# simonamtoft/downsampled-diffusion

Measured on AMD Instinct MI355X. Metric: images/sec (T=1000 sampling), 256x256 dDDPM-x3, higher is better.
Workload: dtype f32

## Files before the change

downsampled-diffusion_amd/csrc/attention.hip:

```cpp
#include <cstdlib>

#include "cluster_sync.h"
#include "conv_common.h"

namespace ddk {

constexpr int DH = 32;

constexpr int PART = DH + DH + DH * DH;

__global__ __launch_bounds__(256) void linattn_context_kernel(const float* __restrict__ qkv, float* __restrict__ ctx,
                                                              float* __restrict__ part, int HW, int heads, int splits, int rows_per_split,
                                                              int kv_only) {
    __shared__ __attribute__((aligned(16))) float stage[4 * 32 * 33];
    float* kexp = stage;
    float* vs = stage + 64 * DH;
    __shared__ float smax[8 * DH];
    const int bh = blockIdx.x / splits, sp = blockIdx.x % splits;
    const int b = bh / heads, h = bh % heads;
    const int HC = heads * DH, RS = (kv_only ? 2 : 3) * HC;
    const float* base = qkv + (long long)b * HW * RS;
    const float* kp = base + (kv_only ? 0 : HC) + h * DH;
    const float* vp = kp + HC;
    const int tid = threadIdx.x;
// ... 1138 lines not shown
        for (int r = 0; r < 16; ++r) Ab[((r & 3) + 8 * (r >> 2) + 4 * kh) * FOLD_C] = acc[r];
        if (tid < 32) {
            float u1 = 0.f, u2 = 0.f;
#pragma unroll 16
            for (int he = 0; he < FOLD_C; ++he) {
                u1 += Wq[tid * (FOLD_C + 1) + he] * t1[he];
                u2 += Wq[tid * (FOLD_C + 1) + he] * t2[he];
            }
            const int n = nq * 32 + tid;
            a1[(long long)b * FOLD_C + n] = u1;
            a2[(long long)b * FOLD_C + n] = u2 + (bout ? bout[n] : 0.f);
        }
    }
}

int linattn_small_qkv_init_device() {
    DDK_HIP(hipFuncSetAttribute(reinterpret_cast<const void*>(attn_kvctx_kernel), hipFuncAttributeMaxDynamicSharedMemorySize,
                                (int)(KC_LDS_FLOATS * sizeof(float))));
    DDK_HIP(hipFuncSetAttribute(reinterpret_cast<const void*>(attn_fold_kernel), hipFuncAttributeMaxDynamicSharedMemorySize,
                                (int)(FOLD_LDS_FLOATS * sizeof(float))));
    DDK_HIP(hipFuncSetAttribute(reinterpret_cast<const void*>(linattn_small_kernel<256>), hipFuncAttributeMaxDynamicSharedMemorySize, 160 * 1024));
    DDK_HIP(hipFuncSetAttribute(reinterpret_cast<const void*>(linattn_small_qkv_kernel<1>), hipFuncAttributeMaxDynamicSharedMemorySize, 160 * 1024));
    DDK_HIP(hipFuncSetAttribute(reinterpret_cast<const void*>(linattn_small_qkv_kernel<4>), hipFuncAttributeMaxDynamicSharedMemorySize, 160 * 1024));
    DDK_HIP(hipFuncSetAttribute(reinterpret_cast<const void*>(attn_split_kernel<128>), hipFuncAttributeMaxDynamicSharedMemorySize,
                                (int)(AttnSplitGeom<128>::LDS_FL * sizeof(float))));
    DDK_HIP(hipFuncSetAttribute(reinterpret_cast<const void*>(attn_split_kernel<32>), hipFuncAttributeMaxDynamicSharedMemorySize,
                                (int)(AttnSplitGeom<32>::LDS_FL * sizeof(float))));
    return DDK_OK;
}

// ... 17 lines not shown
    else
        hipLaunchKernelGGL(linattn_small_qkv_kernel<4>, dim3(B * heads), dim3(256), small_qkv_lds_bytes(4, C), st, x, wop, c1, c2, ln_eps, ctx, out,
                           HW, C, heads);
    return check_launch("linattn_small_qkv_kernel");
}

bool attn_kvctx_ok(int B, int HW, int C, int heads) { return B > 0 && C == KC_K && heads == 4 && HW >= 4 * KC_BM && HW % KC_BM == 0; }
int attn_kvctx_splits(int B, int HW) {
    const int tiles = HW / KC_BM;
    int s = 1;
    while (s * 2 <= tiles && tiles % (s * 2) == 0 && (long long)B * 2 * (s * 2) <= 256) s *= 2;
    return s;
}
size_t attn_kvctx_workspace_bytes(int B, int HW) { return (size_t)B * 4 * attn_kvctx_splits(B, HW) * PART * sizeof(float); }

int attn_kvctx(const float* x, const float* w_kv, const float* c1, const float* c2, float ln_eps, float* ctx, int B, int HW, void* workspace,
               size_t workspace_bytes, hipStream_t st) {
    DDK_REQUIRE(x && w_kv && c1 && c2 && ctx && workspace, "attn_kvctx: null pointer");
    DDK_REQUIRE(attn_kvctx_ok(B, HW, KC_K, 4), "attn_kvctx: needs 128 channels, 4 heads, H*W a multiple of 64 and >= 256");
    DDK_REQUIRE(aligned16(x) && aligned16(w_kv) && aligned16(c1) && aligned16(c2) && aligned16(ctx) && aligned16(workspace), "attn_kvctx: alignment");
    DDK_REQUIRE((long long)B * HW * KC_K * 4 < (1LL << 32) && B <= 65535, "attn_kvctx: input of 4 GiB or more, or more than 65535 images");
    const int s = attn_kvctx_splits(B, HW);
    if (workspace_bytes < attn_kvctx_workspace_bytes(B, HW)) {
        set_error("attn_kvctx: workspace too small (%zu < %zu)", workspace_bytes, attn_kvctx_workspace_bytes(B, HW));
        return DDK_ERR_WORKSPACE;
    }
    DDK_TRY(ensure_device_init());
    KvCtxParams p{x, w_kv, c1, c2, ln_eps, static_cast<float*>(workspace), HW / KC_BM, HW / KC_BM / s, s};
    hipLaunchKernelGGL(attn_kvctx_kernel, dim3((unsigned)s, 2, (unsigned)B), dim3(512), KC_LDS_FLOATS * sizeof(float), st, p);
    DDK_TRY(check_launch("attn_kvctx_kernel"));
    hipLaunchKernelGGL(linattn_merge_kernel, dim3(B * 4), dim3(256), 0, st, static_cast<const float*>(workspace), ctx, s);
    return check_launch("linattn_merge_kernel");
}

constexpr int AS_CUS = 256;
bool attn_split_ok(int B, int HW, int C, int heads) {
    return B > 0 && (HW == 64 || HW == 256) && C >= 32 && C <= 256 && C % 32 == 0 && heads == 4 && 8 * (long long)B <= AS_CUS &&
           conv_wino_cluster_device_ok();
}
size_t attn_split_counter_words(int B) { return (size_t)B * 4 * AS_CNT; }
size_t attn_split_record_floats(int B) { return (size_t)B * 4 * 2 * AS_REC; }
size_t attn_split_workspace_bytes(int B) { return B > 0 ? (32 + attn_split_counter_words(B) + attn_split_record_floats(B)) * sizeof(float) : 0; }
unsigned attention_cluster_timeouts() { return cl_timeouts_read(); }

int attn_split(const float* x, const float* w, const float* c1, const float* c2, float ln_eps, float* ctx, float* out, int B, int HW, int C,
               unsigned* counters, float* records, unsigned* fail, hipStream_t st) {
// ... 10 lines not shown
}

bool attn_fold_ok(int C, int heads) { return C == FOLD_C && heads * DH == FOLD_C; }
size_t attn_fold_out_floats(int B) { return (size_t)B * (FOLD_C * FOLD_C + 2 * FOLD_C); }

int attn_fold(const float* ctx, const float* wqg, const float* c1q, const float* c2q, const float* wout, const float* bout, float* A,
              float* a1, float* a2, int B, int C, int heads, hipStream_t st) {
    DDK_REQUIRE(ctx && wqg && c1q && c2q && wout && A && a1 && a2 && B > 0, "attn_fold: arguments");
    DDK_REQUIRE(attn_fold_ok(C, heads), "attn_fold: C == 128 and heads * 32 == 128 only");
    DDK_REQUIRE(aligned16(ctx) && aligned16(wout) && aligned16(A), "attn_fold: alignment");
    DDK_TRY(ensure_device_init());
    hipLaunchKernelGGL(attn_fold_kernel, dim3(B, 4), dim3(256), FOLD_LDS_FLOATS * sizeof(float), st, ctx, wqg, c1q, c2q, wout, bout, A, a1, a2);
    return check_launch("attn_fold_kernel");
}

int linattn_apply(const float* qkv, const float* ctx, float* out, int B, int HW, int heads, hipStream_t st) {
    DDK_REQUIRE(qkv && ctx && out && B > 0 && HW > 0, "linattn_apply: arguments");
    DDK_REQUIRE(heads >= 1 && heads <= 8, "linattn_apply: heads must be in 1..8");
    DDK_REQUIRE(aligned16(qkv) && aligned16(ctx) && aligned16(out), "linattn_apply: alignment");
    const int tiles = (int)ceil_div(HW, 64);
    const size_t lds = (size_t)heads * 64 * 33 * sizeof(float);
    hipLaunchKernelGGL(linattn_apply_kernel, dim3(B * tiles), dim3(64 * heads), lds, st, qkv, ctx, out, HW, heads, tiles);
    return check_launch("linattn_apply_kernel");
}

}

extern "C" {
size_t ddk_linattn_context_workspace_bytes(int B, int HW, int heads) { return ddk::linattn_context_workspace_bytes(B, HW, heads); }
int ddk_linattn_context(const float* qkv, float* ctx, int B, int HW, int heads, void* workspace, size_t workspace_bytes, ddk_stream_t s) {
    return ddk::linattn_context(qkv, ctx, B, HW, heads, workspace, workspace_bytes, ddk::as_stream(s), false);
}
int ddk_linattn_context_kv(const float* kv, float* ctx, int B, int HW, int heads, void* workspace, size_t workspace_bytes, ddk_stream_t s) {
    return ddk::linattn_context(kv, ctx, B, HW, heads, workspace, workspace_bytes, ddk::as_stream(s), true);
}
size_t ddk_attention_kv_context_workspace_bytes(int B, int HW) { return ddk::attn_kvctx_workspace_bytes(B, HW); }
int ddk_attention_kv_context_ok(int B, int HW, int C, int heads) { return ddk::attn_kvctx_ok(B, HW, C, heads) ? 1 : 0; }
int ddk_attention_kv_context(const float* x, const float* w_kv, const float* c1, const float* c2, float ln_eps, float* ctx, int B, int HW,
                             void* workspace, size_t workspace_bytes, ddk_stream_t s) {
    return ddk::attn_kvctx(x, w_kv, c1, c2, ln_eps, ctx, B, HW, workspace, workspace_bytes, ddk::as_stream(s));
}
size_t ddk_attention_split_workspace_bytes(int B) { return ddk::attn_split_workspace_bytes(B); }
int ddk_attention_split_ok(int B, int HW, int C, int heads) { return ddk::attn_split_ok(B, HW, C, heads) ? 1 : 0; }
int ddk_attention_split_from_x(const float* x, const float* w_folded, const float* c1, const float* c2, float ln_eps, float* ctx, float* out,
                               int B, int HW, int C, int heads, void* workspace, size_t workspace_bytes, ddk_stream_t s) {
    using namespace ddk;
    DDK_REQUIRE(workspace && B > 0 && heads == 4, "attention_split_from_x: arguments (4 heads)");
    if (workspace_bytes < attn_split_workspace_bytes(B)) {
        set_error("attention_split_from_x: workspace too small (%zu < %zu)", workspace_bytes, attn_split_workspace_bytes(B));
        return DDK_ERR_WORKSPACE;
    }
    unsigned* words = static_cast<unsigned*>(workspace);
    return attn_split(x, w_folded, c1, c2, ln_eps, ctx, out, B, HW, C, words + 32, static_cast<float*>(workspace) + 32 + attn_split_counter_words(B),
                      words, as_stream(s));
}
// ... 19 lines not shown
```

downsampled-diffusion_amd/csrc/ddk_internal.h:

```cpp
#pragma once
#include <hip/hip_runtime.h>

#include <cstdarg>
#include <cstddef>
#include <cstdint>
#include <cstdio>

#include "ddk.h"

#ifdef DDK_HOST_SANITIZE
#include "host_sanitize.h"
#endif

namespace ddk {

void set_error(const char* fmt, ...);

inline int fail_arg(const char* what) {
    set_error("bad argument: %s", what);
    return DDK_ERR_ARG;
}

inline int check_launch(const char* what) {
    hipError_t e = hipGetLastError();
// ... 197 lines not shown
int groupnorm_mish_generic(const float* x, const float* gamma, const float* beta, const float* temb, int temb_stride, const float* addend,
                           float* out, int B, int HW, int CP, int C, int groups, float eps, hipStream_t st, const long long* temb_rows = nullptr);
int chan_layernorm_generic(const float* x, const float* g, const float* b, float* out, long long M, int CP, int C, float eps, hipStream_t st);
int unary(int op, const float* x, float* out, long long n, hipStream_t st);
int add(const float* a, const float* b, float* out, long long n, hipStream_t st);
int avgpool2(const float* x, float* out, int B, int H, int W, int C, hipStream_t st);
int upsample_nearest2(const float* x, float* out, int B, int H, int W, int C, hipStream_t st);
size_t linattn_context_workspace_bytes(int B, int HW, int heads);
int linattn_context(const float* qkv, float* ctx, int B, int HW, int heads, void* workspace, size_t workspace_bytes, hipStream_t st,
                    bool kv_only = false);
bool attn_fold_ok(int C, int heads);
bool attn_kvctx_ok(int B, int HW, int C, int heads);
size_t attn_kvctx_workspace_bytes(int B, int HW);
int attn_kvctx(const float* x, const float* w_kv, const float* c1, const float* c2, float ln_eps, float* ctx, int B, int HW, void* workspace,
               size_t workspace_bytes, hipStream_t st);
size_t attn_fold_out_floats(int B);
int attn_fold(const float* ctx, const float* wqg, const float* c1q, const float* c2q, const float* wout, const float* bout, float* A,
              float* a1, float* a2, int B, int C, int heads, hipStream_t st);
int linattn_apply(const float* qkv, const float* ctx, float* out, int B, int HW, int heads, hipStream_t st);
int linattn_fused_small(const float* qkv, float* ctx, float* out, int B, int HW, int heads, hipStream_t st);
bool attn_split_ok(int B, int HW, int C, int heads);
size_t attn_split_counter_words(int B);
size_t attn_split_record_floats(int B);
int attn_split(const float* x, const float* w, const float* c1, const float* c2, float ln_eps, float* ctx, float* out, int B, int HW, int C,
               unsigned* counters, float* records, unsigned* fail, hipStream_t st);
bool linattn_small_qkv_ok(int HW, int C);
int linattn_small_qkv_init_device();
int qkv_operand_pack(const float* lnw, float* wop, int heads, int cp, hipStream_t st);
int linattn_small_qkv(const float* x, const float* wop, const float* c1, const float* c2, float ln_eps, float* ctx, float* out, int B, int HW,
                      int C, int heads, hipStream_t st);
// ... 164 lines not shown
```

downsampled-diffusion_amd/csrc/unet_plan.hip:

```cpp
#include <algorithm>
#include <initializer_list>
#include <mutex>
#include <string>
#include <vector>

#include "ddk_internal.h"
#include "level_chain.h"

namespace ddk {

constexpr int HEADS = 4;
constexpr int HIDDEN = HEADS * 32;
constexpr int GROUPS = 8;
constexpr float GN_EPS = 1e-5f, LN_EPS = 1e-5f;

static inline int pad32(int c) { return (c + 31) / 32 * 32; }

enum PackKind { PK_COPY = 0, PK_CONV = 1, PK_CONVT = 2, PK_LINEAR_T = 3, PK_WINO = 4, PK_LOCAL = 5, PK_WLOCAL = 6, PK_FIRST = 7, PK_CONVT_WINO = 8,
                PK_ROWS = 9 , PK_LOCAL1 = 10 ,
                PK_CONVT_LOCAL = 11 ,
                PK_SKIP_WINO = 12  };

struct Slot {
    std::string name;
// ... 76 lines not shown
    std::vector<SamplerGraph> graphs;
    unsigned long long use_clock = 0;
    unsigned long long pack_epoch = 0;
    struct {
        const void* ws = nullptr;
        int t_start = -1, B = 0, H = 0, W = 0;
        unsigned long long pack_epoch = 0;
        std::vector<int64_t> map;
    } table;
    ddk_unet_config cfg;
    int cluster_gn = 1;
    int cluster_limit = 1 << 30;
    int cluster_np_max = 8;
    bool cluster_split = true;
    bool attn_kvctx = true;
    bool attn_split = true;
    bool skip_fold = true;
    bool fold_down_reduce = false;
    bool restore_fused = true;
    bool first_gn = true;
    int level_chain = 9;
    int level_chain_max_batch = 32;
    int attn_fold_min_hw = 256;
    bool attn_fold = true;
    bool generic = false;
    std::vector<int> dimp;
    std::vector<Slot> slots;
    size_t packed_floats = 0;
    int L = 0;
    std::vector<int> dims;
// ... 278 lines not shown

extern "C" int ddk_unet_set_option(ddk_unet* u, int option, int value) {
    DDK_REQUIRE(u, "unet_set_option: null plan");
    static const struct {
        int option;
        bool drops_graphs;
        void (*set)(ddk_unet&, int);
    } options[] = {
        {DDK_OPT_CLUSTER_GROUPNORM, true, [](ddk_unet& p, int v) { p.cluster_gn = v < 0 ? 0 : v > 2 ? 2 : v; }},
        {DDK_OPT_ATTENTION_FOLD, true, [](ddk_unet& p, int v) { p.attn_fold = v != 0; }},
        {DDK_OPT_ATTENTION_KV_CONTEXT, true, [](ddk_unet& p, int v) { p.attn_kvctx = v != 0; }},
        {DDK_OPT_FIRST_GROUPNORM, true, [](ddk_unet& p, int v) { p.first_gn = v != 0; }},
        {DDK_OPT_RESTORE_FUSED_TAIL, true, [](ddk_unet& p, int v) { p.restore_fused = v != 0; }},
        {DDK_OPT_ATTENTION_SPLIT, true, [](ddk_unet& p, int v) { p.attn_split = v != 0; }},
        {DDK_OPT_SKIP_FOLD, true, [](ddk_unet& p, int v) { p.skip_fold = v != 0; }},
        {DDK_OPT_LEVEL_CHAIN, true, [](ddk_unet& p, int v) {
             p.level_chain = v == 1 ? 9 : v == 2 ? 1 : v == 3 ? 15 : v == 4 ? 6 : v == 8 ? 2 : v == 16 ? 4 : v != 0 ? 9 : 0;
         }},
        {DDK_OPT_FOLD_DOWNSAMPLE_REDUCE, true, [](ddk_unet& p, int v) { p.fold_down_reduce = v != 0; }},
        {10, true, [](ddk_unet& p, int v) { p.level_chain_max_batch = v; }},
        {9, true, [](ddk_unet& p, int v) { p.attn_fold_min_hw = v; }},
        {2, false, [](ddk_unet& p, int v) { p.cluster_limit = v; }},
        {4, true, [](ddk_unet& p, int v) { p.cluster_np_max = v; }},
        {11, true, [](ddk_unet& p, int v) { p.cluster_split = v != 0; }},
    };
    for (const auto& o : options) {
        if (o.option != option) continue;
        std::lock_guard<std::mutex> lock(u->mu);
        if (o.drops_graphs) {
            if (!u->graphs.empty()) DDK_HIP(hipDeviceSynchronize());
// ... 456 lines not shown
    return u.attn_fold && H * W > u.attn_fold_min_hw && (H * W) % 64 == 0 && attn_fold_ok(a.c, HEADS) && conv1x1_ws_ok(M, a.c, a.c) &&
           conv_ln_fold_ok(B, H, W, a.c, 2 * HIDDEN) && B <= 256;
}

static int run_attn(Ctx& c, const AttnW& a, const float* x, float* out, int H, int W) {
    float* xn = c.W + c.ly.off_xn;
    float* qkv = c.W + c.ly.off_qkv;
    float* ctx = c.W + c.ly.off_ctx;
    float* o = c.W + c.ly.off_o;
    const long long M = (long long)c.B * H * W;
    if (!c.u.generic && H * W <= 16 && a.c % 32 == 0 && linattn_small_qkv_ok(H * W, a.c)) {
        DDK_TRY(linattn_small_qkv(x, c.P + a.qkv_op, c.P + a.ln_c1, c.P + a.ln_c2, LN_EPS, ctx, o, c.B, H * W, a.c, HEADS, c.st));
        return run_conv(c, DDK_CONV1X1, a.out, o, HIDDEN, nullptr, 0, x, out, H, W, a.c);
    }
    if (!c.u.generic && attn_fold_eligible(c.u, a, c.B, H, W)) {
        if (c.u.attn_kvctx && attn_kvctx_ok(c.B, H * W, a.c, HEADS) && c.ly.splitk * sizeof(float) >= attn_kvctx_workspace_bytes(c.B, H * W)) {
            DDK_TRY(attn_kvctx(x, c.P + a.qkv_lnw + (size_t)HIDDEN * a.c, c.P + a.ln_c1 + HIDDEN, c.P + a.ln_c2 + HIDDEN, LN_EPS, ctx, c.B, H * W,
                               c.W + c.ly.off_splitk, c.ly.splitk * sizeof(float), c.st));
        } else {
            const ConvLnFold lnkv{c.P + a.ln_c1 + HIDDEN, c.P + a.ln_c2 + HIDDEN, LN_EPS};
            DDK_TRY(run_conv(c, DDK_CONV1X1, a.qkv, x, a.c, nullptr, 0, nullptr, qkv, H, W, 2 * HIDDEN, c.P + a.qkv_lnw + (size_t)HIDDEN * a.c,
                             &lnkv));
            DDK_TRY(linattn_context(qkv, ctx, c.B, H * W, HEADS, c.W + c.ly.off_splitk, c.ly.splitk * sizeof(float), c.st, true));
        }
        float* A = o;
        float* a1 = A + (size_t)c.B * a.c * a.c;
        float* a2 = a1 + (size_t)c.B * a.c;
        DDK_TRY(attn_fold(ctx, c.P + a.qkv_lnw, c.P + a.ln_c1, c.P + a.ln_c2, c.P + a.out.w, a.out.has_bias ? c.P + a.out.b : nullptr, A, a1,
                          a2, c.B, a.c, HEADS, c.st));
        const ConvLnFold lnA{a1, a2, LN_EPS};
        return conv1x1_ws(x, A, nullptr, x, out, M, a.c, &lnA, c.st, c.B);
    }
    if (!c.u.generic && c.u.attn_split && c.allow_cluster && a.c >= 128 && attn_split_ok(c.B, H * W, a.c, HEADS)) {
        float* cl = c.W + c.ly.off_cl;
        DDK_TRY(attn_split(x, c.P + a.qkv_lnw, c.P + a.ln_c1, c.P + a.ln_c2, LN_EPS, ctx, o, c.B, H * W, a.c,
                           reinterpret_cast<unsigned*>(cl + cl_attn_offset(c.B)), cl + cl_counter_floats(c.B), cl_words(cl, c.B).fail, c.st));
        return run_conv(c, DDK_CONV1X1, a.out, o, HIDDEN, nullptr, 0, x, out, H, W, a.c);
    }
    if (!c.u.generic && conv_ln_fold_ok(c.B, H, W, a.c, 3 * HIDDEN)) {
        const ConvLnFold ln{c.P + a.ln_c1, c.P + a.ln_c2, LN_EPS};
        DDK_TRY(run_conv(c, DDK_CONV1X1, a.qkv, x, a.c, nullptr, 0, nullptr, qkv, H, W, 3 * HIDDEN, c.P + a.qkv_lnw, &ln));
    } else {
        DDK_TRY(c.u.generic ? chan_layernorm_generic(x, c.P + a.ln.g, c.P + a.ln.b, xn, M, a.c, a.c_real, LN_EPS, c.st)
                            : chan_layernorm(x, c.P + a.ln.g, c.P + a.ln.b, xn, M, a.c, LN_EPS, c.st));
        DDK_TRY(run_conv(c, DDK_CONV1X1, a.qkv, xn, a.c, nullptr, 0, nullptr, qkv, H, W, 3 * HIDDEN));
// ... 408 lines not shown
        if (k.wino) return 2.0 * (double)(ceil_div((long long)B * (H / 2) * (W / 2), 32) * 32) * 16.0 * cin * N;
        return 2.0 * B * H * W * 9.0 * cin * N;
    };
    auto res = [&](const ResW& r, int H, int W, int c0, int c1, bool fast) {
        if (fast) {
            f += 2.0 * B * H * W * (2.0 * ((9 * r.ci + 1) / 2)) * r.co;
            f += 2.0 * B * H * W * (double)r.ci * r.co;
        } else {
            f += conv3(r.c1, H, W, c0, c1, r.co);
            if (r.has_res) f += conv_flops(DDK_CONV1X1, B, H, W, c0 + c1, r.co);
        }
        f += conv3(r.c2, H, W, r.co, 0, r.co);
    };
    auto attn = [&](const AttnW& a, int H, int W) {
        if (attn_fold_eligible(*u, a, B, H, W)) {
            f += conv_flops(DDK_CONV1X1, B, H, W, a.c, 2 * HIDDEN) + 2.0 * B * HEADS * 32.0 * 32.0 * H * W;
            f += 2.0 * B * (4.0 * HIDDEN * 32.0 * a.c + (double)a.c * HIDDEN * a.c) + conv_flops(DDK_CONV1X1, B, H, W, a.c, a.c);
            return;
        }
        f += conv_flops(DDK_CONV1X1, B, H, W, a.c, 3 * HIDDEN) + conv_flops(DDK_CONV1X1, B, H, W, HIDDEN, a.c);
        f += 2.0 * 2.0 * B * HEADS * 32.0 * 32.0 * H * W;
    };
    int H = H0, W = W0, cur_c = pad32(u->cfg.in_ch);
    for (int l = 0; l < u->L; ++l) {
        const int co = u->dims[l + 1];
        res(u->down_res[2 * l], H, W, cur_c, 0, l == 0 && first_fast(*u, B, H, W));
        res(u->down_res[2 * l + 1], H, W, co, 0, false);
        attn(u->down_attn[l], H, W);
        if (l < u->L - 1) { f += conv_flops(DDK_CONV3X3_S2, B, H, W, co, co); H /= 2; W /= 2; }
        cur_c = co;
    }
    res(u->mid1, H, W, cur_c, 0, false); attn(u->mid_attn, H, W); res(u->mid2, H, W, cur_c, 0, false);
// ... 707 lines not shown
```

downsampled-diffusion_amd/ddk/lib.py:

```python
import ctypes as C
import os

import torch

_HERE = os.path.dirname(os.path.abspath(__file__))
LIB_PATH = os.environ.get("DDK_LIB", os.path.join(os.path.dirname(_HERE), "csrc", "libddk.so"))


class DDKError(RuntimeError):
    pass


ABI_VERSION = 400
ERR_CLUSTER = -4


class ConvArgs(C.Structure):
    _fields_ = [
        ("kind", C.c_int), ("src0", C.c_void_p), ("src1", C.c_void_p), ("c0", C.c_int), ("c1", C.c_int),
        ("weight", C.c_void_p), ("bias", C.c_void_p), ("resid", C.c_void_p), ("out", C.c_void_p),
        ("B", C.c_int), ("H", C.c_int), ("W", C.c_int), ("N", C.c_int), ("pre_mish", C.c_int), ("post_mish", C.c_int), ("defer_reduce", C.c_int),
        ("workspace", C.c_void_p), ("workspace_bytes", C.c_size_t), ("weight_wino", C.c_void_p),
        ("gn_partials", C.c_void_p), ("gn_groups", C.c_int), ("mish_out", C.c_void_p), ("dmish_src", C.c_void_p),
        ("skip_weight", C.c_void_p), ("skip_bias", C.c_void_p), ("skip_out", C.c_void_p), ("skip_slab_stride", C.c_longlong),
# ... 80 lines not shown
    "ddk_conv1x1_ws_images": (_I, [_P, _P, _P, _P, _P, C.c_longlong, _I, _P, _P, _F, _I, _P]),
    "ddk_linattn_context_kv": (_I, [_P, _P, _I, _I, _I, _P, _SZ, _P]),
    "ddk_attention_fold": (_I, [_P, _P, _P, _P, _P, _P, _P, _P, _P, _I, _I, _I, _P]),
    "ddk_groupnorm_mish_partials_res1x1": (_I, [_P, _P, _I, _P, _P, _P, _I, _P, _P, _P, _I, _P, _I, _I, _I, _I, _F, _P]),
    "ddk_final_tail": (_I, [_P, _P, _I, _P, _P, _F, _P, _P, _I, _P, _P, _P, _P, _P, _P, _P, _P, _P, C.c_uint64, C.c_uint32, _I, _I, _I, _I, _P]),
    "ddk_pack_conv_weight_local": (_I, [_P, _P, _I, _I, _I, _P]),
    "ddk_pack_conv1x1_weight_local": (_I, [_P, _P, _I, _I, _I, _P]),
    "ddk_pack_convT_weight_local": (_I, [_P, _P, _I, _I, _P]),
    "ddk_pack_conv_weight_wino_local": (_I, [_P, _P, _I, _I, _I, _P]),
    "ddk_conv3x3_gn_mish_wino_ok": (_I, [_I, _I, _I, _I, _I, _I]),
    "ddk_conv3x3_gn_mish_wino": (_I, [_P, _I, _P, _I, _P, _P, _P, _P, _P, _I, _P, _P, _I, _I, _I, _I, _I, _F, _P]),
    "ddk_conv3x3_gn_mish_slabs": (_I, [_P, _I, _LL, _P, _I, _P, _P, _P, _P, _P, _I, _P, _I, _LL, _P, _P, _I, _I, _I, _I, _I, _F, _P]),
    "ddk_attention_kv_context_workspace_bytes": (_SZ, [_I, _I]),
    "ddk_attention_kv_context_ok": (_I, [_I, _I, _I, _I]),
    "ddk_attention_kv_context": (_I, [_P, _P, _P, _P, _F, _P, _I, _I, _P, _SZ, _P]),
    "ddk_attention_split_workspace_bytes": (_SZ, [_I]),
    "ddk_attention_split_ok": (_I, [_I, _I, _I, _I]),
    "ddk_attention_split_from_x": (_I, [_P, _P, _P, _P, _F, _P, _P, _I, _I, _I, _I, _P, _SZ, _P]),
    "ddk_pack_qkv_operand": (_I, [_P, _P, _I, _I, _P]),
    "ddk_linattn_small_from_x": (_I, [_P, _P, _P, _P, _F, _P, _P, _I, _I, _I, _I, _P]),
    "ddk_conv3x3_gn_mish_ok": (_I, [_I, _I, _I, _I, _I, _I]),
    "ddk_conv3x3_gn_mish": (_I, [_P, _I, _P, _I, _P, _P, _P, _P, _P, _I, _P, _P, _I, _I, _I, _I, _I, _F, _P]),
    "ddk_conv_workspace_bytes": (_SZ, [_I, _I, _I, _I, _I, _I]),
    "ddk_conv_splits": (_I, [_I, _I, _I, _I, _I, _I]),
    "ddk_conv_forward": (_I, [C.POINTER(ConvArgs), _P]),
    "ddk_debug_read_stamps": (_I, [_P]),
    "ddk_groupnorm_mish": (_I, [_P, _P, _P, _P, _I, _P, _P, _I, _I, _I, _I, _F, _P, _SZ, _P]),
    "ddk_groupnorm_workspace_bytes": (_SZ, [_I, _I, _I, _I]),
    "ddk_groupnorm_mish_slabs": (_I, [_P, _I, _LL, _P, _P, _P, _P, _I, _P, _P, _I, _I, _I, _I, _F, _P]),
    "ddk_chan_layernorm": (_I, [_P, _P, _P, _P, _LL, _I, _F, _P]),
# ... 221 lines not shown
```

downsampled-diffusion_amd/ddk/ops.py:

```python
import ctypes as C
import math

import torch

from . import lib as L

CONV3X3_S1, CONV3X3_S2, CONV1X1, CONVT4X4_S2 = 0, 1, 2, 3
GN_GROUPS, GN_EPS, LN_EPS = 8, 1e-5, 1e-5


def pad32(c):
    return (c + 31) // 32 * 32


class _PackEntry:
    __slots__ = ("wref", "out", "job", "fresh", "pooled")


_pack_cache = {}
_weights_epoch = [0]
_pack_table = {}
pack_stats = {"single": 0, "batched_launches": 0, "batched_jobs": 0}
_graph_tables = []
_graph_keep = [_graph_tables]
# ... 363 lines not shown
    lib = L.load()
    if not lib.ddk_attention_kv_context_ok(b, h * w_, c, heads):
        raise L.DDKError(f"attention_kv_context: shape {tuple(x.shape)} with {heads} heads not eligible (C = 128, 4 heads, H*W % 64 == 0)")
    wq = w_qkv.reshape(3 * hc, c).to(torch.float32)
    g, be = ln_g.reshape(-1).to(torch.float32), ln_b.reshape(-1).to(torch.float32)
    wkv = (wq * g.view(1, c))[hc:].contiguous()
    c1, c2 = (wq @ g)[hc:].contiguous(), (wq @ be)[hc:].contiguous()
    ctx = torch.empty((b, heads, 32, 32), device=x.device, dtype=torch.float32)
    nbytes = lib.ddk_attention_kv_context_workspace_bytes(b, h * w_)
    ws = _ws(x.device, nbytes, "kvctx")
    L.check(lib.ddk_attention_kv_context(L.ptr(_f32(x)), L.ptr(wkv), L.ptr(c1), L.ptr(c2), eps, L.ptr(ctx), b, h * w_, L.ptr(ws), nbytes,
                                         L.stream()), "attention_kv_context")
    return ctx


def groupnorm_mish_from_partials_res1x1(x, part, tiles_per_image, gamma, beta, res_x, res_w, res_b, temb=None, groups=GN_GROUPS,
                                        eps=GN_EPS):
    b, h, w_, n = x.shape
    cin = res_x.shape[-1]
    out = torch.empty_like(x)
    stride = temb.stride(0) if temb is not None else 0
    L.check(L.load().ddk_groupnorm_mish_partials_res1x1(
        L.ptr(_f32(x)), L.ptr(part), tiles_per_image, L.ptr(gamma), L.ptr(beta), temb.data_ptr() if temb is not None else None, stride,
        L.ptr(_f32(res_x)), L.ptr(res_w.reshape(n, cin).contiguous()), L.ptr(res_b), cin, L.ptr(out), b, h * w_, n, groups, eps,
        L.stream()), "groupnorm_mish_partials_res1x1")
    return out


def final_tail(raw, part, tiles_per_image, gamma, beta, w, bias, x=None, t=None, tables=None, noise=None, seed=0, stream_id=0,
               want_eps=True, groups=GN_GROUPS, eps=GN_EPS):
# ... 1482 lines not shown
```

downsampled-diffusion_amd/ddk/plan.py:

```python
import contextlib
import ctypes as C
import math
import types
import warnings

import torch

from . import lib as L


def sinusoidal_freqs(dim):
    half = dim // 2
    step = math.log(10000) / (half - 1)
    return torch.exp(torch.arange(half) * -step)


SAMPLERS = {"smp": ("sample", "sampler", "sampler"), "sms": ("sample_multistep", "sampler_multistep", "multistep sampler"),
            "sin": ("sample_inpaint", "sampler_inpaint", "inpainting sampler"),
            "srs": ("sample_restore", "sampler_restore", "super-resolution sampler"),
            "srm": ("sample_restore_masked", "sampler_restore_masked", "masked restoration sampler"),
            "srx": ("sample_restore_multistep", "sampler_restore_multistep", "restoration solver"),
            "srn": ("sample_restore_noisy", "sampler_restore_noisy", "noisy restoration sampler"),
            "srg": ("sample_restore_gray", "sampler_restore_gray", "colourisation sampler"),
            "srb": ("sample_restore_blur", "sampler_restore_blur", "deblurring sampler"),
# ... 69 lines not shown
            for k in [k for k in self._ws if k[0] == kind]:
                del self._ws[k]
        buf = torch.empty(max(nbytes, 16) // 4 + 4, device=device, dtype=torch.float32)
        self._ws[key] = buf
        return buf

    OPT_CLUSTER_GROUPNORM = 1
    OPT_ATTENTION_FOLD = 3
    OPT_FOLD_DOWNSAMPLE_REDUCE = 5
    OPT_ATTENTION_KV_CONTEXT = 6
    OPT_LEVEL_CHAIN = 7
    OPT_FIRST_GROUPNORM = 8
    OPT_RESTORE_FUSED_TAIL = 12
    OPT_ATTENTION_SPLIT = 13
    OPT_SKIP_FOLD = 14

    def set_option(self, option, value):
        L.check(self._lib.ddk_unet_set_option(self.handle, option, int(value)), "unet_set_option")
        if option == self.OPT_CLUSTER_GROUPNORM:
            self._cluster = max(0, min(2, int(value)))

    @contextlib.contextmanager
    def forwards_as_in_chain(self):
        raised = self._cluster == 1
        if raised:
            self.set_option(self.OPT_CLUSTER_GROUPNORM, 2)
        try:
            yield
        finally:
            if raised and self._cluster == 2:
# ... 364 lines not shown
```

include/ddk.h:

```cpp
#ifndef DDK_H
#define DDK_H

#include <stddef.h>
#include <stdint.h>

#ifdef __cplusplus
extern "C" {
#endif

typedef void* ddk_stream_t;

#define DDK_OK 0
#define DDK_ERR_ARG (-1)
#define DDK_ERR_HIP (-2)
#define DDK_ERR_WORKSPACE (-3)
#define DDK_ERR_CLUSTER (-4)

int ddk_version(void);
const char* ddk_last_error(void);
int ddk_device_ok(void);

int ddk_nchw_to_nhwc(const float* src, float* dst, int B, int C, int H, int W, int c_pad, ddk_stream_t s);
int ddk_nhwc_to_nchw(const float* src, float* dst, int B, int C, int H, int W, int c_stride, ddk_stream_t s);
int ddk_pad_channels(const float* src, float* dst, long long M, int C, int c_pad, ddk_stream_t s);
// ... 105 lines not shown
int ddk_mish(const float* x, float* out, long long n, ddk_stream_t s);
int ddk_tanh(const float* x, float* out, long long n, ddk_stream_t s);
int ddk_avgpool2(const float* x, float* out, int B, int H, int W, int C, ddk_stream_t s);
int ddk_upsample_nearest2(const float* x, float* out, int B, int H, int W, int C, ddk_stream_t s);
int ddk_add(const float* a, const float* b, float* out, long long n, ddk_stream_t s);

size_t ddk_linattn_context_workspace_bytes(int B, int HW, int heads);
int ddk_linattn_context(const float* qkv, float* ctx, int B, int HW, int heads, void* workspace, size_t workspace_bytes, ddk_stream_t s);
int ddk_linattn_context_kv(const float* kv, float* ctx, int B, int HW, int heads, void* workspace, size_t workspace_bytes, ddk_stream_t s);
int ddk_attention_fold(const float* ctx, const float* wqg, const float* c1q, const float* c2q, const float* wout, const float* bout, float* A,
                       float* a1, float* a2, int B, int C, int heads, ddk_stream_t s);
size_t ddk_attention_kv_context_workspace_bytes(int B, int HW);
int ddk_attention_kv_context_ok(int B, int HW, int C, int heads);
int ddk_attention_kv_context(const float* x, const float* w_kv, const float* c1, const float* c2, float ln_eps, float* ctx, int B, int HW,
                             void* workspace, size_t workspace_bytes, ddk_stream_t s);
size_t ddk_attention_split_workspace_bytes(int B);
int ddk_attention_split_ok(int B, int HW, int C, int heads);
int ddk_attention_split_from_x(const float* x, const float* w_folded, const float* c1, const float* c2, float ln_eps, float* ctx, float* out,
                               int B, int HW, int C, int heads, void* workspace, size_t workspace_bytes, ddk_stream_t s);
int ddk_linattn_fused_small(const float* qkv, float* ctx, float* out, int B, int HW, int heads, ddk_stream_t s);
int ddk_linattn_apply(const float* qkv, const float* ctx, float* out, int B, int HW, int heads, ddk_stream_t s);
int ddk_pack_qkv_operand(const float* folded_w, float* dst, int heads, int c_pad, ddk_stream_t s);
int ddk_linattn_small_from_x(const float* x, const float* w_operand, const float* c1, const float* c2, float ln_eps, float* ctx,
                             float* out, int B, int HW, int C, int heads, ddk_stream_t s);

int ddk_time_mlp(const int64_t* t, const float* freqs, const float* w1t, const float* b1, const float* w2t,
                 const float* b2, float* act, float* raw, int B, int dim, ddk_stream_t s);
int ddk_time_proj(const float* act, const float* wt, const float* bias, float* out, int B, int dim, int n_out,
                  ddk_stream_t s);

// ... 109 lines not shown
size_t ddk_unet_packed_bytes(const ddk_unet* u);
int ddk_unet_pack_slot(const ddk_unet* u, int slot, const float* canonical, void* packed, ddk_stream_t s);
int ddk_unet_finalize_pack(const ddk_unet* u, void* packed, ddk_stream_t s);
size_t ddk_unet_workspace_bytes(const ddk_unet* u, int B, int H, int W);
int ddk_unet_forward(const ddk_unet* u, const void* packed, const float* x, const int64_t* t, float* out,
                     int B, int H, int W, void* workspace, size_t workspace_bytes, ddk_stream_t s);
#define DDK_OPT_CLUSTER_GROUPNORM 1
#define DDK_OPT_ATTENTION_FOLD 3
#define DDK_OPT_FOLD_DOWNSAMPLE_REDUCE 5
#define DDK_OPT_ATTENTION_KV_CONTEXT 6
#define DDK_OPT_LEVEL_CHAIN 7
#define DDK_OPT_FIRST_GROUPNORM 8
#define DDK_OPT_RESTORE_FUSED_TAIL 12
#define DDK_OPT_ATTENTION_SPLIT 13
#define DDK_OPT_SKIP_FOLD 14
int ddk_unet_set_option(ddk_unet* u, int option, int value);
int ddk_unet_cluster_check(const ddk_unet* u, void* workspace, int B, int H, int W, ddk_stream_t s);
unsigned ddk_debug_cluster_timeouts(void);
int ddk_debug_clock_probe(unsigned long long* out, int workgroups, ddk_stream_t s);
int ddk_debug_occupy(int workgroups, int lds_bytes, int microseconds, ddk_stream_t s);
double ddk_unet_flops(const ddk_unet* u, int B, int H, int W);
double ddk_unet_flops_executed(const ddk_unet* u, int B, int H, int W);

typedef struct ddk_sampler_args {
    const ddk_unet* unet;
    const void* packed;
    float* x;
    const float* noise;
    const float* c_recip;
    const float* c_recipm1;
// ... 237 lines not shown
```

Baseline: 27.05.

## Fuse linear-attention split merge into attention fold kernel via partials

Adds a kernel that reads the per-split key/value context partials directly, merges them with a log-sum-exp rescale, and then does the fold that builds the folded output matrix and LayerNorm vectors. This removes the separate merge kernel launch and the round trip of the context tensor through memory. The fold math is also reordered to multiply the output weight by the context first and then by the query weight, which cuts the per-block work. It is on by default behind a new option, at the cost of more register and LDS use per block and a template per split count.

New measurement: 27.32 (median of 6 runs). +1.0%, better.

```diff
diff --git a/downsampled-diffusion_amd/csrc/attention.hip b/downsampled-diffusion_amd/csrc/attention.hip
--- a/downsampled-diffusion_amd/csrc/attention.hip
+++ b/downsampled-diffusion_amd/csrc/attention.hip
@@ -1176,6 +1176,111 @@
     }
 }
 
+constexpr int FP_CT = 34, FP_PP = FOLD_C + 2;
+template <int S>
+__global__ __launch_bounds__(256) void attn_fold_parts_kernel(const float* __restrict__ part, const float* __restrict__ wqg,
+                                                              const float* __restrict__ c1q, const float* __restrict__ c2q,
+                                                              const float* __restrict__ wout, const float* __restrict__ bout,
+                                                              float* __restrict__ A, float* __restrict__ a1, float* __restrict__ a2) {
+    __shared__ float ctxT[4 * DH * FP_CT];
+    __shared__ float Ps[32 * FP_PP];
+    const int b = blockIdx.x, nq = blockIdx.y, tid = threadIdx.x, lane = tid & 63;
+    const int wave = __builtin_amdgcn_readfirstlane(tid >> 6);
+    const int l31 = lane & 31, kh = lane >> 5;
+    float bw[FOLD_C / 2];
+#pragma unroll
+    for (int s2 = 0; s2 < FOLD_C / 2; ++s2) bw[s2] = wqg[(2 * s2 + kh) * FOLD_C + wave * 32 + l31];
+    float aw[DH / 2];
+#pragma unroll
+    for (int q = 0; q < 4; ++q) {
+        const float4 v = *reinterpret_cast<const float4*>(wout + (long long)(nq * 32 + l31) * FOLD_C + wave * DH + kh * 16 + 4 * q);
+        aw[4 * q] = v.x; aw[4 * q + 1] = v.y; aw[4 * q + 2] = v.z; aw[4 * q + 3] = v.w;
+    }
+    const int vn = tid >> 3, vp = tid & 7;
+    float cv1[FOLD_C / 8], cv2[FOLD_C / 8];
+#pragma unroll
+    for (int i = 0; i < FOLD_C / 8; ++i) {
+        cv1[i] = c1q[8 * i + vp];
+        cv2[i] = c2q[8 * i + vp];
+    }
+    const float bo = bout ? bout[nq * 32 + vn] : 0.f;
+    const float* pp = part + ((long long)b * 4 + wave) * S * PART;
+    const int dl = lane >> 3, e0 = (lane & 7) * 4;
+    float mv[S][4], dv[S][4];
+    float4 rv[S][4];
+#pragma unroll
+    for (int s = 0; s < S; ++s)
+#pragma unroll
+        for (int j = 0; j < 4; ++j) {
+            const int d = dl + 8 * j;
+            mv[s][j] = pp[s * PART + d];
+            dv[s][j] = pp[s * PART + DH + d];
+            rv[s][j] = *reinterpret_cast<const float4*>(pp + s * PART + 2 * DH + d * DH + e0);
+        }
+    __builtin_amdgcn_sched_barrier(0);
+#pragma unroll
+    for (int j = 0; j < 4; ++j) {
+        const int d = dl + 8 * j;
+        float M = -INFINITY;
+#pragma unroll
+        for (int s = 0; s < S; ++s) M = fmaxf(M, mv[s][j]);
+        float4 acc = make_float4(0.f, 0.f, 0.f, 0.f);
+        float den = 0.f;
+#pragma unroll
+        for (int s = 0; s < S; ++s) {
+            const float w = expf(mv[s][j] - M);
+            const float4 a = rv[s][j];
+            den += dv[s][j] * w;
+            acc.x += a.x * w; acc.y += a.y * w; acc.z += a.z * w; acc.w += a.w * w;
+        }
+        const float inv = 1.0f / den;
+        acc.x *= inv; acc.y *= inv; acc.z *= inv; acc.w *= inv;
+        float* ct = ctxT + (wave * DH + e0) * FP_CT + d;
+        ct[0] = acc.x; ct[FP_CT] = acc.y; ct[2 * FP_CT] = acc.z; ct[3 * FP_CT] = acc.w;
+    }
+    __syncthreads();
+    {
+        f32x16_att acc;
+#pragma unroll
+        for (int r = 0; r < 16; ++r) acc[r] = 0.f;
+#pragma unroll
+        for (int s2 = 0; s2 < DH / 2; ++s2)
+            acc = __builtin_amdgcn_mfma_f32_32x32x2f32(aw[s2], ctxT[(wave * DH + kh * 16 + s2) * FP_CT + l31], acc, 0, 0, 0);
+#pragma unroll
+        for (int r = 0; r < 16; ++r) Ps[((r & 3) + 8 * (r >> 2) + 4 * kh) * FP_PP + wave * DH + l31] = acc[r];
+    }
+    __syncthreads();
+    {
+        f32x16_att acc;
+#pragma unroll
+        for (int r = 0; r < 16; ++r) acc[r] = 0.f;
+#pragma unroll
+        for (int s2 = 0; s2 < FOLD_C / 2; ++s2) acc = __builtin_amdgcn_mfma_f32_32x32x2f32(Ps[l31 * FP_PP + 2 * s2 + kh], bw[s2], acc, 0, 0, 0);
+        float* Ab = A + ((long long)b * FOLD_C + nq * 32) * FOLD_C + wave * 32 + l31;
+#pragma unroll
+        for (int r = 0; r < 16; ++r) Ab[((r & 3) + 8 * (r >> 2) + 4 * kh) * FOLD_C] = acc[r];
+    }
+    {
+        float u1 = 0.f, u2 = 0.f;
+#pragma unroll
+        for (int i = 0; i < FOLD_C / 8; ++i) {
+            const float p = Ps[vn * FP_PP + 8 * i + vp];
+            u1 += p * cv1[i];
+            u2 += p * cv2[i];
+        }
+#pragma unroll
+        for (int m = 1; m < 8; m *= 2) {
+            u1 += __shfl_xor(u1, m, 64);
+            u2 += __shfl_xor(u2, m, 64);
+        }
+        if (vp == 0) {
+            const int n = nq * 32 + vn;
+            a1[(long long)b * FOLD_C + n] = u1;
+            a2[(long long)b * FOLD_C + n] = u2 + bo;
+        }
+    }
+}
+
 int linattn_small_qkv_init_device() {
     DDK_HIP(hipFuncSetAttribute(reinterpret_cast<const void*>(attn_kvctx_kernel), hipFuncAttributeMaxDynamicSharedMemorySize,
                                 (int)(KC_LDS_FLOATS * sizeof(float))));
@@ -1223,11 +1328,11 @@
 }
 size_t attn_kvctx_workspace_bytes(int B, int HW) { return (size_t)B * 4 * attn_kvctx_splits(B, HW) * PART * sizeof(float); }
 
-int attn_kvctx(const float* x, const float* w_kv, const float* c1, const float* c2, float ln_eps, float* ctx, int B, int HW, void* workspace,
-               size_t workspace_bytes, hipStream_t st) {
-    DDK_REQUIRE(x && w_kv && c1 && c2 && ctx && workspace, "attn_kvctx: null pointer");
+int attn_kvctx_parts(const float* x, const float* w_kv, const float* c1, const float* c2, float ln_eps, int B, int HW, void* workspace,
+                     size_t workspace_bytes, hipStream_t st) {
+    DDK_REQUIRE(x && w_kv && c1 && c2 && workspace, "attn_kvctx: null pointer");
     DDK_REQUIRE(attn_kvctx_ok(B, HW, KC_K, 4), "attn_kvctx: needs 128 channels, 4 heads, H*W a multiple of 64 and >= 256");
-    DDK_REQUIRE(aligned16(x) && aligned16(w_kv) && aligned16(c1) && aligned16(c2) && aligned16(ctx) && aligned16(workspace), "attn_kvctx: alignment");
+    DDK_REQUIRE(aligned16(x) && aligned16(w_kv) && aligned16(c1) && aligned16(c2) && aligned16(workspace), "attn_kvctx: alignment");
     DDK_REQUIRE((long long)B * HW * KC_K * 4 < (1LL << 32) && B <= 65535, "attn_kvctx: input of 4 GiB or more, or more than 65535 images");
     const int s = attn_kvctx_splits(B, HW);
     if (workspace_bytes < attn_kvctx_workspace_bytes(B, HW)) {
@@ -1237,8 +1342,22 @@
     DDK_TRY(ensure_device_init());
     KvCtxParams p{x, w_kv, c1, c2, ln_eps, static_cast<float*>(workspace), HW / KC_BM, HW / KC_BM / s, s};
     hipLaunchKernelGGL(attn_kvctx_kernel, dim3((unsigned)s, 2, (unsigned)B), dim3(512), KC_LDS_FLOATS * sizeof(float), st, p);
-    DDK_TRY(check_launch("attn_kvctx_kernel"));
-    hipLaunchKernelGGL(linattn_merge_kernel, dim3(B * 4), dim3(256), 0, st, static_cast<const float*>(workspace), ctx, s);
+    return check_launch("attn_kvctx_kernel");
+}
+
+int attn_kvctx(const float* x, const float* w_kv, const float* c1, const float* c2, float ln_eps, float* ctx, int B, int HW, void* workspace,
+               size_t workspace_bytes, hipStream_t st) {
+    DDK_REQUIRE(ctx && aligned16(ctx), "attn_kvctx: ctx null or misaligned");
+    DDK_TRY(attn_kvctx_parts(x, w_kv, c1, c2, ln_eps, B, HW, workspace, workspace_bytes, st));
+    hipLaunchKernelGGL(linattn_merge_kernel, dim3(B * 4), dim3(256), 0, st, static_cast<const float*>(workspace), ctx,
+                       attn_kvctx_splits(B, HW));
+    return check_launch("linattn_merge_kernel");
+}
+
+int linattn_merge(const float* part, float* ctx, int B, int heads, int splits, hipStream_t st) {
+    DDK_REQUIRE(part && ctx && B > 0 && heads > 0 && splits > 0, "linattn_merge: arguments");
+    DDK_REQUIRE(aligned16(part) && aligned16(ctx), "linattn_merge: alignment");
+    hipLaunchKernelGGL(linattn_merge_kernel, dim3(B * heads), dim3(256), 0, st, part, ctx, splits);
     return check_launch("linattn_merge_kernel");
 }
 
@@ -1279,6 +1398,28 @@
     return check_launch("attn_fold_kernel");
 }
 
+bool attn_fold_parts_ok(int C, int heads, int splits) {
+    return attn_fold_ok(C, heads) && heads == 4 && (splits == 1 || splits == 2 || splits == 4 || splits == 8);
+}
+template <int S>
+static void attn_fold_parts_launch(const float* part, const float* wqg, const float* c1q, const float* c2q, const float* wout,
+                                   const float* bout, float* A, float* a1, float* a2, int B, hipStream_t st) {
+    hipLaunchKernelGGL(attn_fold_parts_kernel<S>, dim3(B, 4), dim3(256), 0, st, part, wqg, c1q, c2q, wout, bout, A, a1, a2);
+}
+int attn_fold_parts(const float* part, int splits, const float* wqg, const float* c1q, const float* c2q, const float* wout, const float* bout,
+                    float* A, float* a1, float* a2, int B, int C, int heads, hipStream_t st) {
+    DDK_REQUIRE(part && wqg && c1q && c2q && wout && A && a1 && a2 && B > 0, "attn_fold_parts: arguments");
+    DDK_REQUIRE(attn_fold_parts_ok(C, heads, splits), "attn_fold_parts: C == 128, 4 heads and 1, 2, 4 or 8 splits only");
+    DDK_REQUIRE(aligned16(part) && aligned16(wout) && aligned16(A), "attn_fold_parts: alignment");
+    switch (splits) {
+        case 1: attn_fold_parts_launch<1>(part, wqg, c1q, c2q, wout, bout, A, a1, a2, B, st); break;
+        case 2: attn_fold_parts_launch<2>(part, wqg, c1q, c2q, wout, bout, A, a1, a2, B, st); break;
+        case 4: attn_fold_parts_launch<4>(part, wqg, c1q, c2q, wout, bout, A, a1, a2, B, st); break;
+        default: attn_fold_parts_launch<8>(part, wqg, c1q, c2q, wout, bout, A, a1, a2, B, st); break;
+    }
+    return check_launch("attn_fold_parts_kernel");
+}
+
 int linattn_apply(const float* qkv, const float* ctx, float* out, int B, int HW, int heads, hipStream_t st) {
     DDK_REQUIRE(qkv && ctx && out && B > 0 && HW > 0, "linattn_apply: arguments");
     DDK_REQUIRE(heads >= 1 && heads <= 8, "linattn_apply: heads must be in 1..8");
@@ -1304,6 +1445,22 @@
 int ddk_attention_kv_context(const float* x, const float* w_kv, const float* c1, const float* c2, float ln_eps, float* ctx, int B, int HW,
                              void* workspace, size_t workspace_bytes, ddk_stream_t s) {
     return ddk::attn_kvctx(x, w_kv, c1, c2, ln_eps, ctx, B, HW, workspace, workspace_bytes, ddk::as_stream(s));
+}
+int ddk_attention_kv_context_splits(int B, int HW) { return ddk::attn_kvctx_ok(B, HW, ddk::KC_K, 4) ? ddk::attn_kvctx_splits(B, HW) : 0; }
+int ddk_attention_kv_partials(const float* x, const float* w_kv, const float* c1, const float* c2, float ln_eps, int B, int HW, void* workspace,
+                              size_t workspace_bytes, int* splits, ddk_stream_t s) {
+    DDK_REQUIRE(splits, "attention_kv_partials: null split count");
+    DDK_TRY(ddk::attn_kvctx_parts(x, w_kv, c1, c2, ln_eps, B, HW, workspace, workspace_bytes, ddk::as_stream(s)));
+    *splits = ddk::attn_kvctx_splits(B, HW);
+    return DDK_OK;
+}
+int ddk_linattn_merge(const float* part, float* ctx, int B, int heads, int splits, ddk_stream_t s) {
+    return ddk::linattn_merge(part, ctx, B, heads, splits, ddk::as_stream(s));
+}
+int ddk_attention_fold_partials_ok(int C, int heads, int splits) { return ddk::attn_fold_parts_ok(C, heads, splits) ? 1 : 0; }
+int ddk_attention_fold_partials(const float* part, int splits, const float* wqg, const float* c1q, const float* c2q, const float* wout,
+                                const float* bout, float* A, float* a1, float* a2, int B, int C, int heads, ddk_stream_t s) {
+    return ddk::attn_fold_parts(part, splits, wqg, c1q, c2q, wout, bout, A, a1, a2, B, C, heads, ddk::as_stream(s));
 }
 size_t ddk_attention_split_workspace_bytes(int B) { return ddk::attn_split_workspace_bytes(B); }
 int ddk_attention_split_ok(int B, int HW, int C, int heads) { return ddk::attn_split_ok(B, HW, C, heads) ? 1 : 0; }
diff --git a/downsampled-diffusion_amd/csrc/ddk_internal.h b/downsampled-diffusion_amd/csrc/ddk_internal.h
--- a/downsampled-diffusion_amd/csrc/ddk_internal.h
+++ b/downsampled-diffusion_amd/csrc/ddk_internal.h
@@ -235,6 +235,12 @@
 size_t attn_kvctx_workspace_bytes(int B, int HW);
 int attn_kvctx(const float* x, const float* w_kv, const float* c1, const float* c2, float ln_eps, float* ctx, int B, int HW, void* workspace,
                size_t workspace_bytes, hipStream_t st);
+int attn_kvctx_splits(int B, int HW);
+int attn_kvctx_parts(const float* x, const float* w_kv, const float* c1, const float* c2, float ln_eps, int B, int HW, void* workspace,
+                     size_t workspace_bytes, hipStream_t st);
+bool attn_fold_parts_ok(int C, int heads, int splits);
+int attn_fold_parts(const float* part, int splits, const float* wqg, const float* c1q, const float* c2q, const float* wout, const float* bout,
+                    float* A, float* a1, float* a2, int B, int C, int heads, hipStream_t st);
 size_t attn_fold_out_floats(int B);
 int attn_fold(const float* ctx, const float* wqg, const float* c1q, const float* c2q, const float* wout, const float* bout, float* A,
               float* a1, float* a2, int B, int C, int heads, hipStream_t st);
diff --git a/downsampled-diffusion_amd/csrc/unet_plan.hip b/downsampled-diffusion_amd/csrc/unet_plan.hip
--- a/downsampled-diffusion_amd/csrc/unet_plan.hip
+++ b/downsampled-diffusion_amd/csrc/unet_plan.hip
@@ -114,6 +114,7 @@
     int cluster_np_max = 8;
     bool cluster_split = true;
     bool attn_kvctx = true;
+    bool attn_fold_parts = true;
     bool attn_split = true;
     bool skip_fold = true;
     bool fold_down_reduce = false;
@@ -422,6 +423,7 @@
         {DDK_OPT_RESTORE_FUSED_TAIL, true, [](ddk_unet& p, int v) { p.restore_fused = v != 0; }},
         {DDK_OPT_ATTENTION_SPLIT, true, [](ddk_unet& p, int v) { p.attn_split = v != 0; }},
         {DDK_OPT_SKIP_FOLD, true, [](ddk_unet& p, int v) { p.skip_fold = v != 0; }},
+        {DDK_OPT_ATTENTION_FOLD_PARTIALS, true, [](ddk_unet& p, int v) { p.attn_fold_parts = v != 0; }},
         {DDK_OPT_LEVEL_CHAIN, true, [](ddk_unet& p, int v) {
              p.level_chain = v == 1 ? 9 : v == 2 ? 1 : v == 3 ? 15 : v == 4 ? 6 : v == 8 ? 2 : v == 16 ? 4 : v != 0 ? 9 : 0;
          }},
@@ -908,21 +910,28 @@
         return run_conv(c, DDK_CONV1X1, a.out, o, HIDDEN, nullptr, 0, x, out, H, W, a.c);
     }
     if (!c.u.generic && attn_fold_eligible(c.u, a, c.B, H, W)) {
+        float* A = o;
+        float* a1 = A + (size_t)c.B * a.c * a.c;
+        float* a2 = a1 + (size_t)c.B * a.c;
+        const float *wqg = c.P + a.qkv_lnw, *bout = a.out.has_bias ? c.P + a.out.b : nullptr;
+        const ConvLnFold lnA{a1, a2, LN_EPS};
         if (c.u.attn_kvctx && attn_kvctx_ok(c.B, H * W, a.c, HEADS) && c.ly.splitk * sizeof(float) >= attn_kvctx_workspace_bytes(c.B, H * W)) {
-            DDK_TRY(attn_kvctx(x, c.P + a.qkv_lnw + (size_t)HIDDEN * a.c, c.P + a.ln_c1 + HIDDEN, c.P + a.ln_c2 + HIDDEN, LN_EPS, ctx, c.B, H * W,
-                               c.W + c.ly.off_splitk, c.ly.splitk * sizeof(float), c.st));
+            const float *wkv = wqg + (size_t)HIDDEN * a.c, *c1kv = c.P + a.ln_c1 + HIDDEN, *c2kv = c.P + a.ln_c2 + HIDDEN;
+            float* part = c.W + c.ly.off_splitk;
+            const int splits = attn_kvctx_splits(c.B, H * W);
+            if (c.u.attn_fold_parts && attn_fold_parts_ok(a.c, HEADS, splits)) {
+                DDK_TRY(attn_kvctx_parts(x, wkv, c1kv, c2kv, LN_EPS, c.B, H * W, part, c.ly.splitk * sizeof(float), c.st));
+                DDK_TRY(attn_fold_parts(part, splits, wqg, c.P + a.ln_c1, c.P + a.ln_c2, c.P + a.out.w, bout, A, a1, a2, c.B, a.c, HEADS, c.st));
+                return conv1x1_ws(x, A, nullptr, x, out, M, a.c, &lnA, c.st, c.B);
+            }
+            DDK_TRY(attn_kvctx(x, wkv, c1kv, c2kv, LN_EPS, ctx, c.B, H * W, part, c.ly.splitk * sizeof(float), c.st));
         } else {
             const ConvLnFold lnkv{c.P + a.ln_c1 + HIDDEN, c.P + a.ln_c2 + HIDDEN, LN_EPS};
             DDK_TRY(run_conv(c, DDK_CONV1X1, a.qkv, x, a.c, nullptr, 0, nullptr, qkv, H, W, 2 * HIDDEN, c.P + a.qkv_lnw + (size_t)HIDDEN * a.c,
                              &lnkv));
             DDK_TRY(linattn_context(qkv, ctx, c.B, H * W, HEADS, c.W + c.ly.off_splitk, c.ly.splitk * sizeof(float), c.st, true));
         }
-        float* A = o;
-        float* a1 = A + (size_t)c.B * a.c * a.c;
-        float* a2 = a1 + (size_t)c.B * a.c;
-        DDK_TRY(attn_fold(ctx, c.P + a.qkv_lnw, c.P + a.ln_c1, c.P + a.ln_c2, c.P + a.out.w, a.out.has_bias ? c.P + a.out.b : nullptr, A, a1,
-                          a2, c.B, a.c, HEADS, c.st));
-        const ConvLnFold lnA{a1, a2, LN_EPS};
+        DDK_TRY(attn_fold(ctx, wqg, c.P + a.ln_c1, c.P + a.ln_c2, c.P + a.out.w, bout, A, a1, a2, c.B, a.c, HEADS, c.st));
         return conv1x1_ws(x, A, nullptr, x, out, M, a.c, &lnA, c.st, c.B);
     }
     if (!c.u.generic && c.u.attn_split && c.allow_cluster && a.c >= 128 && attn_split_ok(c.B, H * W, a.c, HEADS)) {
@@ -1361,8 +1370,10 @@
     };
     auto attn = [&](const AttnW& a, int H, int W) {
         if (attn_fold_eligible(*u, a, B, H, W)) {
+            const bool parts = u->attn_kvctx && u->attn_fold_parts && attn_kvctx_ok(B, H * W, a.c, HEADS) &&
+                               attn_fold_parts_ok(a.c, HEADS, attn_kvctx_splits(B, H * W));
             f += conv_flops(DDK_CONV1X1, B, H, W, a.c, 2 * HIDDEN) + 2.0 * B * HEADS * 32.0 * 32.0 * H * W;
-            f += 2.0 * B * (4.0 * HIDDEN * 32.0 * a.c + (double)a.c * HIDDEN * a.c) + conv_flops(DDK_CONV1X1, B, H, W, a.c, a.c);
+            f += 2.0 * B * ((parts ? 1.0 : 4.0) * HIDDEN * 32.0 * a.c + (double)a.c * HIDDEN * a.c) + conv_flops(DDK_CONV1X1, B, H, W, a.c, a.c);
             return;
         }
         f += conv_flops(DDK_CONV1X1, B, H, W, a.c, 3 * HIDDEN) + conv_flops(DDK_CONV1X1, B, H, W, HIDDEN, a.c);
diff --git a/downsampled-diffusion_amd/ddk/lib.py b/downsampled-diffusion_amd/ddk/lib.py
--- a/downsampled-diffusion_amd/ddk/lib.py
+++ b/downsampled-diffusion_amd/ddk/lib.py
@@ -118,6 +118,11 @@
     "ddk_attention_kv_context_workspace_bytes": (_SZ, [_I, _I]),
     "ddk_attention_kv_context_ok": (_I, [_I, _I, _I, _I]),
     "ddk_attention_kv_context": (_I, [_P, _P, _P, _P, _F, _P, _I, _I, _P, _SZ, _P]),
+    "ddk_attention_kv_context_splits": (_I, [_I, _I]),
+    "ddk_attention_kv_partials": (_I, [_P, _P, _P, _P, _F, _I, _I, _P, _SZ, C.POINTER(C.c_int), _P]),
+    "ddk_linattn_merge": (_I, [_P, _P, _I, _I, _I, _P]),
+    "ddk_attention_fold_partials_ok": (_I, [_I, _I, _I]),
+    "ddk_attention_fold_partials": (_I, [_P, _I, _P, _P, _P, _P, _P, _P, _P, _P, _I, _I, _I, _P]),
     "ddk_attention_split_workspace_bytes": (_SZ, [_I]),
     "ddk_attention_split_ok": (_I, [_I, _I, _I, _I]),
     "ddk_attention_split_from_x": (_I, [_P, _P, _P, _P, _F, _P, _P, _I, _I, _I, _I, _P, _SZ, _P]),
diff --git a/downsampled-diffusion_amd/ddk/ops.py b/downsampled-diffusion_amd/ddk/ops.py
--- a/downsampled-diffusion_amd/ddk/ops.py
+++ b/downsampled-diffusion_amd/ddk/ops.py
@@ -401,6 +401,45 @@
     return ctx
 
 
+def attention_kv_partials(x, w_qkv, ln_g, ln_b, heads=4, eps=LN_EPS):
+    b, h, w_, c = x.shape
+    hc = heads * 32
+    lib = L.load()
+    if not lib.ddk_attention_kv_context_ok(b, h * w_, c, heads):
+        raise L.DDKError(f"attention_kv_partials: shape {tuple(x.shape)} with {heads} heads not eligible (C = 128, 4 heads, H*W % 64 == 0)")
+    wq = w_qkv.reshape(3 * hc, c).to(torch.float32)
+    g, be = ln_g.reshape(-1).to(torch.float32), ln_b.reshape(-1).to(torch.float32)
+    wkv = (wq * g.view(1, c))[hc:].contiguous()
+    c1, c2 = (wq @ g)[hc:].contiguous(), (wq @ be)[hc:].contiguous()
+    nbytes = lib.ddk_attention_kv_context_workspace_bytes(b, h * w_)
+    part = torch.empty(nbytes // 4, device=x.device, dtype=torch.float32)
+    splits = C.c_int(0)
+    L.check(lib.ddk_attention_kv_partials(L.ptr(_f32(x)), L.ptr(wkv), L.ptr(c1), L.ptr(c2), eps, b, h * w_, L.ptr(part), nbytes,
+                                          C.byref(splits), L.stream()), "attention_kv_partials")
+    return part.view(b, heads, splits.value, 2 * 32 + 32 * 32)
+
+
+def linattn_merge(part):
+    b, heads, splits, _ = part.shape
+    ctx = torch.empty((b, heads, 32, 32), device=part.device, dtype=torch.float32)
+    L.check(L.load().ddk_linattn_merge(L.ptr(_f32(part)), L.ptr(ctx), b, heads, splits, L.stream()), "linattn_merge")
+    return ctx
+
+
+def attention_fold_partials(part, wqg, c1q, c2q, w_out, b_out=None, out=None):
+    b, heads, splits, _ = part.shape
+    c = wqg.shape[1]
+    lib = L.load()
+    if not lib.ddk_attention_fold_partials_ok(c, heads, splits):
+        raise L.DDKError(f"attention_fold_partials: C = {c}, {heads} heads, {splits} splits not eligible (C = 128, 4 heads, 1 / 2 / 4 / 8 splits)")
+    a_mat, a1, a2 = out if out is not None else (torch.empty((b, c, c), device=part.device, dtype=torch.float32),
+                                                 torch.empty((b, c), device=part.device, dtype=torch.float32),
+                                                 torch.empty((b, c), device=part.device, dtype=torch.float32))
+    L.check(lib.ddk_attention_fold_partials(L.ptr(_f32(part)), splits, L.ptr(wqg), L.ptr(c1q), L.ptr(c2q), L.ptr(w_out), L.ptr(b_out),
+                                            L.ptr(a_mat), L.ptr(a1), L.ptr(a2), b, c, heads, L.stream()), "attention_fold_partials")
+    return a_mat, a1, a2
+
+
 def groupnorm_mish_from_partials_res1x1(x, part, tiles_per_image, gamma, beta, res_x, res_w, res_b, temb=None, groups=GN_GROUPS,
                                         eps=GN_EPS):
     b, h, w_, n = x.shape
diff --git a/downsampled-diffusion_amd/ddk/plan.py b/downsampled-diffusion_amd/ddk/plan.py
--- a/downsampled-diffusion_amd/ddk/plan.py
+++ b/downsampled-diffusion_amd/ddk/plan.py
@@ -107,6 +107,7 @@
     OPT_RESTORE_FUSED_TAIL = 12
     OPT_ATTENTION_SPLIT = 13
     OPT_SKIP_FOLD = 14
+    OPT_ATTENTION_FOLD_PARTIALS = 15
 
     def set_option(self, option, value):
         L.check(self._lib.ddk_unet_set_option(self.handle, option, int(value)), "unet_set_option")
diff --git a/include/ddk.h b/include/ddk.h
--- a/include/ddk.h
+++ b/include/ddk.h
@@ -143,6 +143,13 @@
 int ddk_attention_kv_context_ok(int B, int HW, int C, int heads);
 int ddk_attention_kv_context(const float* x, const float* w_kv, const float* c1, const float* c2, float ln_eps, float* ctx, int B, int HW,
                              void* workspace, size_t workspace_bytes, ddk_stream_t s);
+int ddk_attention_kv_context_splits(int B, int HW);
+int ddk_attention_kv_partials(const float* x, const float* w_kv, const float* c1, const float* c2, float ln_eps, int B, int HW,
+                              void* workspace, size_t workspace_bytes, int* splits, ddk_stream_t s);
+int ddk_linattn_merge(const float* part, float* ctx, int B, int heads, int splits, ddk_stream_t s);
+int ddk_attention_fold_partials_ok(int C, int heads, int splits);
+int ddk_attention_fold_partials(const float* part, int splits, const float* wqg, const float* c1q, const float* c2q, const float* wout,
+                                const float* bout, float* A, float* a1, float* a2, int B, int C, int heads, ddk_stream_t s);
 size_t ddk_attention_split_workspace_bytes(int B);
 int ddk_attention_split_ok(int B, int HW, int C, int heads);
 int ddk_attention_split_from_x(const float* x, const float* w_folded, const float* c1, const float* c2, float ln_eps, float* ctx, float* out,
@@ -282,6 +289,7 @@
 #define DDK_OPT_RESTORE_FUSED_TAIL 12
 #define DDK_OPT_ATTENTION_SPLIT 13
 #define DDK_OPT_SKIP_FOLD 14
+#define DDK_OPT_ATTENTION_FOLD_PARTIALS 15
 int ddk_unet_set_option(ddk_unet* u, int option, int value);
 int ddk_unet_cluster_check(const ddk_unet* u, void* workspace, int B, int H, int W, ddk_stream_t s);
 unsigned ddk_debug_cluster_timeouts(void);
```
